# davidfang00/opticalflowdiffusion

Hardware: AMD Instinct MI355X
Metric: UNet denoise steps/sec @ 2x436x1024 flow, bs=16 (higher is better)
Workload: dtype bf16

## Files before the change

### opticalflowdiffusion_amd/build.py

```python
import concurrent.futures as cf
import os
import subprocess
import sys

HERE = os.path.dirname(os.path.abspath(__file__))
CSRC = os.path.join(HERE, "csrc")
OUT_DIR = os.path.join(HERE, "lib")
LIB = os.path.join(OUT_DIR, "libofd_hip.so")
ARCH = "gfx950"

COMMON = ["-O3", "-std=c++17", "-fPIC", f"--offload-arch={ARCH}", "-munsafe-fp-atomics",
          "-Wall", "-Wno-unused-function", "-Wno-unused-variable"]
EXTRA = {f: ["-ffp-contract=off"] for f in ("splat.hip", "grid_warp.hip", "splat_pyramid.hip", "diffusion.hip", "x0_quantile.hip",
                                                "loss_rows.hip")}


def sources():
    return sorted(f for f in os.listdir(CSRC) if f.endswith((".hip", ".cpp")))


def _deps_mtime():
    hdrs = [os.path.join(CSRC, f) for f in os.listdir(CSRC) if f.endswith((".h", ".hpp"))]
    hdrs.append(os.path.join(os.path.dirname(HERE), "include", "ofd.h"))
    return max(os.path.getmtime(h) for h in hdrs)


def _compile(src, force):
    obj = os.path.join(OUT_DIR, "obj", src + ".o")
    path = os.path.join(CSRC, src)
    if (not force and os.path.exists(obj) and os.path.getmtime(obj) > max(os.path.getmtime(path), _deps_mtime())):
        return obj, False
    cmd = ["hipcc", "-x", "hip", "-c", path, "-o", obj] + COMMON + EXTRA.get(src, [])
    r = subprocess.run(cmd, capture_output=True, text=True)
    if r.returncode != 0:
        raise RuntimeError(f"hipcc failed on {src}:\n{r.stdout}\n{r.stderr}")
    if r.stderr.strip():
        sys.stderr.write(r.stderr)
    return obj, True


def build(force=False, verbose=True):
    os.makedirs(os.path.join(OUT_DIR, "obj"), exist_ok=True)
    srcs = sources()
    with cf.ThreadPoolExecutor(max_workers=min(8, len(srcs))) as ex:
        results = list(ex.map(lambda s: _compile(s, force), srcs))
    objs = [o for o, _ in results]
    if any(c for _, c in results) or not os.path.exists(LIB):
        cmd = ["hipcc", "-shared", "-fPIC", f"--offload-arch={ARCH}", "-o", LIB] + objs
        r = subprocess.run(cmd, capture_output=True, text=True)
        if r.returncode != 0:
            raise RuntimeError(f"link failed:\n{r.stdout}\n{r.stderr}")
        if verbose:
            print(f"built {LIB} from {len(objs)} objects")
    return LIB


if __name__ == "__main__":
    build(force="--force" in sys.argv)
```

### opticalflowdiffusion_amd/csrc/blocks.hip

```cpp
#include <cstdlib>
#include "blocks.h"
#include "conv_common.h"

namespace ofd {

__device__ __forceinline__ uint32_t pack2(float a, float b) { return f2bf2(a, b); }
__device__ __forceinline__ void unpack8(const uint4& v, float (&f)[8]) {
    const uint32_t w[4] = {v.x, v.y, v.z, v.w};
#pragma unroll
    for (int j = 0; j < 4; ++j) {
        f[2 * j] = bf2f((bf16_t)(w[j] & 0xffffu));
        f[2 * j + 1] = bf2f((bf16_t)(w[j] >> 16));
    }
}
__device__ __forceinline__ uint4 pack8(const float (&f)[8]) {
    return make_uint4(pack2(f[0], f[1]), pack2(f[2], f[3]), pack2(f[4], f[5]), pack2(f[6], f[7]));
}

template <int CP>
__global__ void __launch_bounds__(256) pack_input_kernel(const float* __restrict__ x, int Cx, const float* __restrict__ cond, int Cc,
                                                         bf16_t* __restrict__ out, int B, size_t plane, int ax, int ac) {
    const size_t total = (size_t)B * plane;
    for (size_t i = (size_t)blockIdx.x * blockDim.x + threadIdx.x; i < total; i += (size_t)gridDim.x * blockDim.x) {
        const size_t n = i / plane, pix = i % plane;
        float v[CP];
#pragma unroll
        for (int c = 0; c < CP; ++c) {
            float t = 0.0f;
            if (c < Cx) { t = x[(n * Cx + c) * plane + pix]; if (ax) t = 2.0f * t - 1.0f; }
            else if (c < Cx + Cc) { t = cond[(n * Cc + (c - Cx)) * plane + pix]; if (ac) t = 2.0f * t - 1.0f; }
            v[c] = t;
        }
        uint4* o = (uint4*)(out + i * CP);
#pragma unroll
        for (int k = 0; k < CP / 8; ++k)
            o[k] = make_uint4(pack2(v[8 * k], v[8 * k + 1]), pack2(v[8 * k + 2], v[8 * k + 3]), pack2(v[8 * k + 4], v[8 * k + 5]), pack2(v[8 * k + 6], v[8 * k + 7]));
    }
}

__global__ void __launch_bounds__(256) time_mlp_kernel(const int64_t* __restrict__ t, const float* __restrict__ w1, const float* __restrict__ b1,
                                                       const float* __restrict__ w2, const float* __restrict__ b2, float* __restrict__ temb,
                                                       float* __restrict__ temb_silu, int dim) {
    __shared__ float emb[256], h1[1024];
    const int b = blockIdx.x, tid = threadIdx.x, tdim = dim * 4, half_dim = dim / 2;
    const float tv = (float)t[b];
    for (int i = tid; i < half_dim; i += 256) {
        const float k = (float)(9.210340371976184 / (double)(half_dim - 1));
        const float f = expf((float)i * -k);
        emb[i] = sinf(tv * f);
        emb[half_dim + i] = cosf(tv * f);
    }
    __syncthreads();
    for (int j = tid; j < tdim; j += 256) {
        float a = b1[j];
        for (int k = 0; k < dim; ++k) a += w1[(size_t)j * dim + k] * emb[k];
        h1[j] = 0.5f * a * (1.0f + erff(a * 0.70710678118654752f));
    }
    __syncthreads();
    for (int j = tid; j < tdim; j += 256) {
        float a = b2[j];
        for (int k = 0; k < tdim; ++k) a += w2[(size_t)j * tdim + k] * h1[k];
        temb[(size_t)b * tdim + j] = a;
        temb_silu[(size_t)b * tdim + j] = a / (1.0f + expf(-a));
    }
}

__global__ void __launch_bounds__(256) block_mlp_kernel(const float* __restrict__ temb_silu, const MlpDesc* __restrict__ descs,
                                                        float* __restrict__ ss, int tdim, int ss_stride) {
    __shared__ float e[1024];
    const int b = blockIdx.x, tid = threadIdx.x;
    const MlpDesc d = descs[blockIdx.y];
    for (int k = tid; k < tdim; k += 256) e[k] = temb_silu[(size_t)b * tdim + k];
    __syncthreads();
    for (int j = tid; j < d.n_out; j += 256) {
        float a = d.bias[j];
        const float* wr = d.weight + (size_t)j * tdim;
        if ((tdim & 3) == 0) {
#pragma unroll 8
            for (int k = 0; k < tdim; k += 4) {
                const float4 w4 = *(const float4*)(wr + k);
                a += w4.x * e[k];
                a += w4.y * e[k + 1];
                a += w4.z * e[k + 2];
                a += w4.w * e[k + 3];
            }
        } else {
            for (int k = 0; k < tdim; ++k) a += wr[k] * e[k];
        }
        ss[(size_t)b * ss_stride + d.offset + j] = a;
    }
}

constexpr int GNF_NT = 1024;
__global__ void __launch_bounds__(GNF_NT) gn_finalize_kernel(const float* __restrict__ partial, int tiles, int C, double count,
                                                          const float* __restrict__ gamma, const float* __restrict__ beta,
                                                          const float* __restrict__ ss, int ss_stride, int ss_offset,
                                                          float* __restrict__ a_out, float* __restrict__ s_out, float* __restrict__ stats_out) {
    const int b = blockIdx.x, g = blockIdx.y, tid = threadIdx.x;
    const int gs = C / 8, octs = gs / 8;
    constexpr int GU = 8;
    double s1 = 0.0, s2 = 0.0;
    const int total = tiles * octs;
    const float2* run = (const float2*)partial + ((size_t)b * 8 + g) * total;
    for (int i0 = tid; i0 < total; i0 += GNF_NT * GU) {
        float2 v[GU];
#pragma unroll
        for (int u = 0; u < GU; ++u) v[u] = run[min(i0 + u * GNF_NT, total - 1)];
#pragma unroll
        for (int u = 0; u < GU; ++u)
            if (i0 + u * GNF_NT < total) { s1 += (double)v[u].x; s2 += (double)v[u].y; }
    }
    for (int o = 32; o > 0; o >>= 1) { s1 += __shfl_xor(s1, o, 64); s2 += __shfl_xor(s2, o, 64); }
    __shared__ double r1[GNF_NT / 64], r2[GNF_NT / 64];
    if ((tid & 63) == 0) { r1[tid >> 6] = s1; r2[tid >> 6] = s2; }
    __syncthreads();
    for (int k = GNF_NT / 128; k > 0; k >>= 1) {
        if (tid < k) { r1[tid] += r1[tid + k]; r2[tid] += r2[tid + k]; }
        __syncthreads();
    }
    const double mean_d = r1[0] / count;
    double var_d = r2[0] / count - mean_d * mean_d;
    if (var_d < 0.0) var_d = 0.0;
    const float mean = (float)mean_d, rstd = rsqrtf((float)var_d + 1e-5f);
    if (stats_out && tid == 0) {
        stats_out[((size_t)b * 8 + g) * 2] = mean;
        stats_out[((size_t)b * 8 + g) * 2 + 1] = rstd;
    }
    for (int c = g * gs + tid; c < (g + 1) * gs; c += GNF_NT) {
        float sc = 0.0f, sh = 0.0f;
        if (ss) {
            sc = ss[(size_t)b * ss_stride + ss_offset + c];
            sh = ss[(size_t)b * ss_stride + ss_offset + C + c];
        }
        const float ga = gamma[c] * rstd;
        a_out[(size_t)b * C + c] = ga * (sc + 1.0f);
        s_out[(size_t)b * C + c] = (beta[c] - mean * ga) * (sc + 1.0f) + sh;
    }
}

__global__ void __launch_bounds__(256) resblock_out_kernel(const bf16_t* __restrict__ h, const float* __restrict__ a, const float* __restrict__ s,
                                                           const bf16_t* __restrict__ x, bf16_t* __restrict__ out, int C, size_t pix_per_sample, size_t total_units) {
    const int c8n = C / 8;
    for (size_t u = (size_t)blockIdx.x * blockDim.x + threadIdx.x; u < total_units; u += (size_t)gridDim.x * blockDim.x) {
        const size_t pix = u / c8n;
        const int c = (int)(u % c8n) * 8;
        const size_t b = pix / pix_per_sample;
        float hv[8], xv[8], av[8], sv[8];
        unpack8(*(const uint4*)(h + u * 8), hv);
        unpack8(*(const uint4*)(x + u * 8), xv);
        *(float4*)&av[0] = *(const float4*)(a + b * C + c);
        *(float4*)&av[4] = *(const float4*)(a + b * C + c + 4);
        *(float4*)&sv[0] = *(const float4*)(s + b * C + c);
        *(float4*)&sv[4] = *(const float4*)(s + b * C + c + 4);
#pragma unroll
        for (int j = 0; j < 8; ++j) hv[j] = silu_f(hv[j] * av[j] + sv[j]) + xv[j];
        *(uint4*)(out + u * 8) = pack8(hv);
    }
}

__global__ void __launch_bounds__(256) layernorm_c_kernel(const bf16_t* __restrict__ x, const float* __restrict__ g, const bf16_t* __restrict__ res,
                                                          bf16_t* __restrict__ out, int C, float eps, size_t npix) {
    const int lpp = C / 8;
    const int lane = threadIdx.x & 63;
    const int sub = lane % lpp, slot = lane / lpp, ppw = 64 / lpp;
    const size_t wave_global = ((size_t)blockIdx.x * blockDim.x + threadIdx.x) >> 6;
    const size_t nwaves = ((size_t)gridDim.x * blockDim.x) >> 6;
    float gv[8];
    *(float4*)&gv[0] = *(const float4*)(g + sub * 8);
    *(float4*)&gv[4] = *(const float4*)(g + sub * 8 + 4);
    const float inv_c = 1.0f / (float)C;
    for (size_t p0 = wave_global * ppw; p0 < npix; p0 += nwaves * ppw) {
        const size_t p = p0 + slot;
        const bool ok = p < npix;
        float v[8];
        if (ok) unpack8(*(const uint4*)(x + p * C + sub * 8), v);
        else {
#pragma unroll
            for (int j = 0; j < 8; ++j) v[j] = 0.0f;
        }
        float s = ((v[0] + v[1]) + (v[2] + v[3])) + ((v[4] + v[5]) + (v[6] + v[7]));
        for (int o = 1; o < lpp; o <<= 1) s += __shfl_xor(s, o, 64);
        const float mean = s * inv_c;
        float q = 0.0f;
#pragma unroll
        for (int j = 0; j < 8; ++j) { v[j] -= mean; q += v[j] * v[j]; }
        for (int o = 1; o < lpp; o <<= 1) q += __shfl_xor(q, o, 64);
        const float rstd = rsqrtf(q * inv_c + eps);
        if (ok) {
            float r[8];
            if (res) unpack8(*(const uint4*)(res + p * C + sub * 8), r);
#pragma unroll
            for (int j = 0; j < 8; ++j) v[j] = v[j] * rstd * gv[j] + (res ? r[j] : 0.0f);
            *(uint4*)(out + p * C + sub * 8) = pack8(v);
        }
    }
}

__global__ void __launch_bounds__(256) la_ctx_combine_kernel(const float* __restrict__ partial, float* __restrict__ ctx, int nparts, float inv_n, float* __restrict__ ml_out) {
    __shared__ float M[32], Linv[32], red[8][32];
    extern __shared__ float w_s[];
    const int tid = threadIdx.x, bh = blockIdx.x, dd = tid & 31, grp = tid >> 5;
    const float* base = partial + (size_t)bh * nparts * 1088;
    float mx = -3.0e38f;
    for (int c = grp; c < nparts; c += 8) mx = fmaxf(mx, base[(size_t)c * 1088 + dd]);
    red[grp][dd] = mx;
    __syncthreads();
    if (tid < 32) {
        float m = red[0][tid];
#pragma unroll
        for (int g = 1; g < 8; ++g) m = fmaxf(m, red[g][tid]);
        M[tid] = m;
    }
    __syncthreads();
    const bool use_ws = nparts <= 256;
    float l = 0.0f;
    for (int c = grp; c < nparts; c += 8) {
        const float w = __expf(base[(size_t)c * 1088 + dd] - M[dd]);
        if (use_ws) w_s[c * 32 + dd] = w;
        l += base[(size_t)c * 1088 + 32 + dd] * w;
    }
    __syncthreads();
    red[grp][dd] = l;
    __syncthreads();
    if (tid < 32) {
        float t = red[0][tid];
#pragma unroll
        for (int g = 1; g < 8; ++g) t += red[g][tid];
        Linv[tid] = 1.0f / t;
        if (ml_out && blockIdx.y == 0) {
            ml_out[(size_t)bh * 64 + tid] = M[tid];
            ml_out[(size_t)bh * 64 + 32 + tid] = 1.0f / t;
        }
    }
    __syncthreads();
    {
        const int i = blockIdx.y * 256 + tid, d = i >> 5;
        float a = 0.0f;
        for (int c0 = 0; c0 < nparts; c0 += 8) {
            float v[8];
#pragma unroll
            for (int k = 0; k < 8; ++k) v[k] = base[(size_t)min(c0 + k, nparts - 1) * 1088 + 64 + i];
            if (use_ws) {
#pragma unroll
                for (int k = 0; k < 8; ++k)
                    if (c0 + k < nparts) a += v[k] * w_s[(c0 + k) * 32 + d];
            } else {
#pragma unroll
                for (int k = 0; k < 8; ++k)
                    if (c0 + k < nparts) a += v[k] * __expf(base[(size_t)(c0 + k) * 1088 + d] - M[d]);
            }
        }
        ctx[(size_t)bh * 1024 + i] = a * Linv[d] * inv_n;
    }
}

constexpr int FA_KT = 64;
__global__ void __launch_bounds__(256) flash_attn_d32_kernel(const bf16_t* __restrict__ qkv, bf16_t* __restrict__ out, int n, float scale, float* __restrict__ lse) {
    __shared__ __attribute__((aligned(16))) unsigned char k_lds[FA_KT * 80];
    __shared__ __attribute__((aligned(16))) unsigned char vt_lds[32 * 144];
    const int tid = threadIdx.x, lane = tid & 63, wave = tid >> 6, l31 = lane & 31, half = lane >> 5;
    const int bh = blockIdx.y, b = bh / 4, h = bh % 4;
    const int q0 = blockIdx.x * 128 + wave * 32;
    const bf16_t* base = qkv + (size_t)b * n * 384;

    bf16x8 qf[2];
    {
        const int q = min(q0 + l31, n - 1);
#pragma unroll
        for (int s = 0; s < 2; ++s) qf[s] = *(const bf16x8*)(base + (size_t)q * 384 + h * 32 + s * 16 + half * 8);
    }
    f32x16 o_acc;
#pragma unroll
    for (int r = 0; r < 16; ++r) o_acc[r] = 0.0f;
    float m_run = -3.0e38f, l_run = 0.0f;

    for (int j0 = 0; j0 < n; j0 += FA_KT) {
        __syncthreads();
        {
            const int key = tid >> 2, u = tid & 3;
            const int kg = min(j0 + key, n - 1);
            const uint4 kv = *(const uint4*)(base + (size_t)kg * 384 + 128 + h * 32 + u * 8);
            *(uint4*)(k_lds + key * 80 + u * 16) = kv;
            const uint4 vv = *(const uint4*)(base + (size_t)kg * 384 + 256 + h * 32 + u * 8);
            const int kb = key >> 5, kk = key & 31, s = kk >> 4, a = (kk >> 3) & 1, hh = (kk >> 2) & 1, bb = kk & 3;
            const int slot = kb * 32 + s * 16 + hh * 8 + a * 4 + bb;
            const uint32_t w[4] = {vv.x, vv.y, vv.z, vv.w};
#pragma unroll
            for (int j = 0; j < 4; ++j) {
                *(bf16_t*)(vt_lds + (u * 8 + 2 * j) * 144 + slot * 2) = (bf16_t)(w[j] & 0xffffu);
                *(bf16_t*)(vt_lds + (u * 8 + 2 * j + 1) * 144 + slot * 2) = (bf16_t)(w[j] >> 16);
            }
        }
        __syncthreads();
        f32x16 s_acc[2];
#pragma unroll
        for (int kb = 0; kb < 2; ++kb) {
#pragma unroll
            for (int r = 0; r < 16; ++r) s_acc[kb][r] = 0.0f;
#pragma unroll
            for (int s = 0; s < 2; ++s) {
                const bf16x8 kf = *(const bf16x8*)(k_lds + (kb * 32 + l31) * 80 + (s * 16 + half * 8) * 2);
                s_acc[kb] = __builtin_amdgcn_mfma_f32_32x32x16_bf16(kf, qf[s], s_acc[kb], 0, 0, 0);
            }
        }
        if (j0 + FA_KT > n) {
#pragma unroll
            for (int kb = 0; kb < 2; ++kb)
#pragma unroll
                for (int r = 0; r < 16; ++r)
                    if (j0 + kb * 32 + (r & 3) + 8 * (r >> 2) + 4 * half >= n) s_acc[kb][r] = -3.0e38f;
        }
        float mx = -3.0e38f;
#pragma unroll
        for (int kb = 0; kb < 2; ++kb)
#pragma unroll
            for (int r = 0; r < 16; ++r) mx = fmaxf(mx, s_acc[kb][r]);
        mx = fmaxf(mx, __shfl_xor(mx, 32, 64));
        const float m_new = fmaxf(m_run, mx);
        const float c = scale * 1.4426950408889634f, m2 = m_new * c;
        const float alpha = __builtin_amdgcn_exp2f(__builtin_fmaf(m_run, c, -m2));
        m_run = m_new;
        float psum = 0.0f;
#pragma unroll
        for (int kb = 0; kb < 2; ++kb)
#pragma unroll
            for (int r = 0; r < 16; ++r) {
                const float p = __builtin_amdgcn_exp2f(__builtin_fmaf(s_acc[kb][r], c, -m2));
                s_acc[kb][r] = p;
                psum += p;
            }
        l_run = l_run * alpha + psum;
#pragma unroll
        for (int r = 0; r < 16; ++r) o_acc[r] *= alpha;
#pragma unroll
        for (int kb = 0; kb < 2; ++kb)
#pragma unroll
            for (int s = 0; s < 2; ++s) {
                bf16x8 pf;
#pragma unroll
                for (int j = 0; j < 8; ++j) pf[j] = (__bf16)s_acc[kb][8 * s + j];
                const bf16x8 vf = *(const bf16x8*)(vt_lds + l31 * 144 + (kb * 32 + s * 16 + half * 8) * 2);
                o_acc = __builtin_amdgcn_mfma_f32_32x32x16_bf16(vf, pf, o_acc, 0, 0, 0);
            }
    }
    const float l_tot = l_run + __shfl_xor(l_run, 32, 64);
    const float inv = 1.0f / l_tot;
    const int q = q0 + l31;
    if (lse && q < n && half == 0) lse[(size_t)bh * n + q] = m_run * scale + __logf(l_tot);
    if (q < n) {
        bf16_t* dst = out + ((size_t)b * n + q) * 128 + h * 32;
#pragma unroll
        for (int g = 0; g < 4; ++g) {
            const uint2 pk = make_uint2(pack2(o_acc[4 * g] * inv, o_acc[4 * g + 1] * inv), pack2(o_acc[4 * g + 2] * inv, o_acc[4 * g + 3] * inv));
            *(uint2*)(dst + 8 * g + 4 * half) = pk;
        }
    }
}

__device__ __forceinline__ float clamp1(float v) { return v < -1.0f ? -1.0f : (v > 1.0f ? 1.0f : v); }
__device__ __forceinline__ float out_glue(float v, int mode, float div) {
    if (mode == 1) return clamp1(clamp1(v) / div);
    if (mode == 2) return (clamp1(v) + 1.0f) / 2.0f;
    return v;
}

template <int OD>
__global__ void __launch_bounds__(256) final_conv_kernel(const bf16_t* __restrict__ x, const float* __restrict__ w, const float* __restrict__ bias,
                                                         float* __restrict__ out, int C, int out_dim, size_t plane, size_t total, int out_mode,
                                                         float out_div) {
    const int lpp = C / 8, lane = threadIdx.x & 63, sub = lane % lpp, slot = lane / lpp, ppw = 64 / lpp;
    float wv[OD][8];
#pragma unroll
    for (int o = 0; o < OD; ++o)
#pragma unroll
        for (int j = 0; j < 8; ++j) wv[o][j] = (o < out_dim) ? w[o * C + sub * 8 + j] : 0.0f;
    const size_t wave_global = ((size_t)blockIdx.x * blockDim.x + threadIdx.x) >> 6, nwaves = ((size_t)gridDim.x * blockDim.x) >> 6;
    for (size_t p0 = wave_global * ppw; p0 < total; p0 += nwaves * ppw) {
        const size_t i = min(p0 + slot, total - 1);
        float f[8];
        unpack8(*(const uint4*)(x + i * C + sub * 8), f);
        float acc[OD];
#pragma unroll
        for (int o = 0; o < OD; ++o) {
            acc[o] = 0.0f;
#pragma unroll
            for (int j = 0; j < 8; ++j) acc[o] += f[j] * wv[o][j];
            for (int k = 1; k < lpp; k <<= 1) acc[o] += __shfl_xor(acc[o], k, 64);
        }
        if (OD == 4) {
            if (sub < out_dim && p0 + slot < total) {
                const size_t n = i / plane, pix = i % plane;
                float r = acc[0];
                if (sub == 1) r = acc[1];
                if (sub == 2) r = acc[2];
                if (sub == 3) r = acc[3];
                out[(n * out_dim + sub) * plane + pix] = out_glue(r + bias[sub], out_mode, out_div);
            }
        } else if (p0 + slot < total) {
            const size_t n = i / plane, pix = i % plane;
#pragma unroll
            for (int o = 0; o < OD; ++o)
                if (o < out_dim && o % lpp == sub) out[(n * out_dim + o) * plane + pix] = out_glue(acc[o] + bias[o], out_mode, out_div);
        }
    }
}

__global__ void __launch_bounds__(256) nhwc_to_nchw_kernel(const bf16_t* __restrict__ x, float* __restrict__ out, int C, size_t plane, size_t total) {
    for (size_t i = (size_t)blockIdx.x * blockDim.x + threadIdx.x; i < total; i += (size_t)gridDim.x * blockDim.x) {
        const size_t pixc = i / C;
        const int c = (int)(i % C);
        const size_t n = pixc / plane, pix = pixc % plane;
        out[(n * C + c) * plane + pix] = bf2f(x[i]);
    }
}
__global__ void __launch_bounds__(256) nchw_to_nhwc_kernel(const float* __restrict__ x, bf16_t* __restrict__ out, int C, size_t plane, size_t total) {
    for (size_t i = (size_t)blockIdx.x * blockDim.x + threadIdx.x; i < total; i += (size_t)gridDim.x * blockDim.x) {
        const size_t pixc = i / C;
        const int c = (int)(i % C);
        const size_t n = pixc / plane, pix = pixc % plane;
        out[i] = f2bf(x[(n * C + c) * plane + pix]);
    }
}

static inline int sgrid(size_t total, int block = 256, int cap = 4096) {
    if (cap <= 0) cap = 1 << 22;
    size_t b = (total + block - 1) / block;
    return (int)(b < 1 ? 1 : (b > (size_t)cap ? cap : b));
}

int k_pack_input(const float* x, int Cx, const float* cond, int Cc, bf16_t* out, int B, int H, int W, hipStream_t s, int cpad, int ax, int ac) {
    OFD_CHECK_ARG((cpad == 8 || cpad == 16 || cpad == 32 || cpad == 48) && Cx + Cc <= cpad && Cx > 0, "pack_input: %d+%d channels into %d", Cx, Cc, cpad);
    const int g = sgrid((size_t)B * H * W);
    const size_t plane = (size_t)H * W;
    if (cpad == 8) pack_input_kernel<8><<<g, 256, 0, s>>>(x, Cx, cond, Cc, out, B, plane, ax, ac);
    else if (cpad == 16) pack_input_kernel<16><<<g, 256, 0, s>>>(x, Cx, cond, Cc, out, B, plane, ax, ac);
    else if (cpad == 32) pack_input_kernel<32><<<g, 256, 0, s>>>(x, Cx, cond, Cc, out, B, plane, ax, ac);
    else pack_input_kernel<48><<<g, 256, 0, s>>>(x, Cx, cond, Cc, out, B, plane, ax, ac);
    OFD_LAUNCH_CHECK();
    return OFD_OK;
}
int k_time_mlp(const int64_t* t, const float* w1, const float* b1, const float* w2, const float* b2, float* temb, float* temb_silu, int B, int dim, hipStream_t s) {
    OFD_CHECK_ARG(dim * 4 <= 1024 && dim <= 256, "time_mlp: dim %d too large", dim);
    time_mlp_kernel<<<B, 256, 0, s>>>(t, w1, b1, w2, b2, temb, temb_silu, dim);
    OFD_LAUNCH_CHECK();
    return OFD_OK;
}
int k_block_mlp(const float* temb_silu, const MlpDesc* descs, int n_desc, float* ss, int B, int tdim, int ss_stride, hipStream_t s) {
    block_mlp_kernel<<<dim3(B, n_desc), 256, 0, s>>>(temb_silu, descs, ss, tdim, ss_stride);
    OFD_LAUNCH_CHECK();
    return OFD_OK;
}
int k_gn_finalize(const float* partial, int B, int H, int W, int C, const float* gamma, const float* beta, const float* ss, int ss_stride,
                  int ss_offset, float* a_out, float* s_out, hipStream_t s, float* stats_out) {
    OFD_CHECK_ARG(C % 64 == 0, "gn_finalize: C=%d", C);
    const int tiles = cdiv(H, 8) * cdiv(W, 32) * 4;
    gn_finalize_kernel<<<dim3(B, 8), GNF_NT, 0, s>>>(partial, tiles, C, (double)H * W * (C / 8), gamma, beta, ss, ss_stride, ss_offset, a_out, s_out, stats_out);
    OFD_LAUNCH_CHECK();
    return OFD_OK;
}
int k_resblock_out(const bf16_t* h, const float* a, const float* sft, const bf16_t* x, bf16_t* out, int B, int H, int W, int C, hipStream_t s) {
    const size_t units = (size_t)B * H * W * (C / 8);
    resblock_out_kernel<<<sgrid(units, 256, 0), 256, 0, s>>>(h, a, sft, x, out, C, (size_t)H * W, units);
    OFD_LAUNCH_CHECK();
    return OFD_OK;
}
int k_layernorm_c(const bf16_t* x, const float* g, const bf16_t* res, bf16_t* out, size_t npix, int C, float eps, hipStream_t s) {
    OFD_CHECK_ARG(C == 64 || C == 128 || C == 256 || C == 512, "layernorm_c: C=%d unsupported", C);
    const size_t waves = (npix + (512 / C) - 1) / (512 / C);
    layernorm_c_kernel<<<sgrid(waves * 64, 256, 0), 256, 0, s>>>(x, g, res, out, C, eps, npix);
    OFD_LAUNCH_CHECK();
    return OFD_OK;
}
void launch_la_ctx_combine(const float* partial, float* ctx, int B, int nparts, float inv_n, float* ml_out, hipStream_t s) {
    const size_t lds = (size_t)(nparts <= 256 ? nparts : 1) * 32 * sizeof(float);
    la_ctx_combine_kernel<<<dim3(B * 4, 4), 256, lds, s>>>(partial, ctx, nparts, inv_n, ml_out);
}
int k_flash_attention(const bf16_t* qkv, bf16_t* out, int B, int n, hipStream_t s, float* lse) {
    flash_attn_d32_kernel<<<dim3(cdiv(n, 128), B * 4), 256, 0, s>>>(qkv, out, n, 0.17677669529663687f, lse);
    OFD_LAUNCH_CHECK();
    return OFD_OK;
}
int k_final_conv(const bf16_t* x, const float* w, const float* bias, float* out, int B, int H, int W, int C, int out_dim, hipStream_t s, int out_mode,
                 float out_div) {
    OFD_CHECK_ARG(out_dim >= 1 && out_dim <= 16 && C % 8 == 0, "final_conv: out_dim=%d C=%d", out_dim, C);
    OFD_CHECK_ARG(C == 64 || C == 128 || C == 256 || C == 512, "final_conv: C=%d unsupported", C);
    OFD_CHECK_ARG(out_mode >= 0 && out_mode <= 2 && out_div > 0.0f, "final_conv: out_mode=%d out_div=%g", out_mode, (double)out_div);
    const int g = sgrid(((size_t)B * H * W + (512 / C) - 1) / (512 / C) * 64);
    if (out_dim <= 4) final_conv_kernel<4><<<g, 256, 0, s>>>(x, w, bias, out, C, out_dim, (size_t)H * W, (size_t)B * H * W, out_mode, out_div);
    else final_conv_kernel<16><<<g, 256, 0, s>>>(x, w, bias, out, C, out_dim, (size_t)H * W, (size_t)B * H * W, out_mode, out_div);
    OFD_LAUNCH_CHECK();
    return OFD_OK;
}
int k_nhwc_to_nchw(const bf16_t* x, float* out, int B, int H, int W, int C, hipStream_t s) {
    const size_t total = (size_t)B * H * W * C;
    nhwc_to_nchw_kernel<<<sgrid(total), 256, 0, s>>>(x, out, C, (size_t)H * W, total);
    OFD_LAUNCH_CHECK();
    return OFD_OK;
}
int k_nchw_to_nhwc(const float* x, bf16_t* out, int B, int H, int W, int C, hipStream_t s) {
    const size_t total = (size_t)B * H * W * C;
    nchw_to_nhwc_kernel<<<sgrid(total), 256, 0, s>>>(x, out, C, (size_t)H * W, total);
    OFD_LAUNCH_CHECK();
    return OFD_OK;
}

}
```

Measured before the change: 34.31.

## Rewrite flash attention with double-buffered 128-key tiles and multi-query-block waves

Moves the d=32 flash attention kernel into its own file and restructures it. Key and value tiles are 128 keys wide and double-buffered in LDS, with global loads for the next tile issued before the current compute. That leaves one barrier per tile instead of two per 64 keys. V is stored in a permuted layout and read with a transpose-fragment helper instead of scalar transposing stores. Each wave can optionally process two 32-query blocks to reuse the K/V fragments, the rescale of the accumulator is skipped when the running max is unchanged, and P is packed to bf16 pairs directly. This adds LDS footprint and register pressure, and the grid-size heuristic picks NB=2 only in a narrow range.

```diff
diff --git a/opticalflowdiffusion_amd/build.py b/opticalflowdiffusion_amd/build.py
--- a/opticalflowdiffusion_amd/build.py
+++ b/opticalflowdiffusion_amd/build.py
@@ -13,6 +13,7 @@
           "-Wall", "-Wno-unused-function", "-Wno-unused-variable"]
 EXTRA = {f: ["-ffp-contract=off"] for f in ("splat.hip", "grid_warp.hip", "splat_pyramid.hip", "diffusion.hip", "x0_quantile.hip",
                                                 "loss_rows.hip")}
+EXTRA["flash_attn.hip"] = ["-fno-slp-vectorize"]
 
 
 def sources():
diff --git a/opticalflowdiffusion_amd/csrc/blocks.hip b/opticalflowdiffusion_amd/csrc/blocks.hip
--- a/opticalflowdiffusion_amd/csrc/blocks.hip
+++ b/opticalflowdiffusion_amd/csrc/blocks.hip
@@ -254,109 +254,6 @@
     }
 }
 
-constexpr int FA_KT = 64;
-__global__ void __launch_bounds__(256) flash_attn_d32_kernel(const bf16_t* __restrict__ qkv, bf16_t* __restrict__ out, int n, float scale, float* __restrict__ lse) {
-    __shared__ __attribute__((aligned(16))) unsigned char k_lds[FA_KT * 80];
-    __shared__ __attribute__((aligned(16))) unsigned char vt_lds[32 * 144];
-    const int tid = threadIdx.x, lane = tid & 63, wave = tid >> 6, l31 = lane & 31, half = lane >> 5;
-    const int bh = blockIdx.y, b = bh / 4, h = bh % 4;
-    const int q0 = blockIdx.x * 128 + wave * 32;
-    const bf16_t* base = qkv + (size_t)b * n * 384;
-
-    bf16x8 qf[2];
-    {
-        const int q = min(q0 + l31, n - 1);
-#pragma unroll
-        for (int s = 0; s < 2; ++s) qf[s] = *(const bf16x8*)(base + (size_t)q * 384 + h * 32 + s * 16 + half * 8);
-    }
-    f32x16 o_acc;
-#pragma unroll
-    for (int r = 0; r < 16; ++r) o_acc[r] = 0.0f;
-    float m_run = -3.0e38f, l_run = 0.0f;
-
-    for (int j0 = 0; j0 < n; j0 += FA_KT) {
-        __syncthreads();
-        {
-            const int key = tid >> 2, u = tid & 3;
-            const int kg = min(j0 + key, n - 1);
-            const uint4 kv = *(const uint4*)(base + (size_t)kg * 384 + 128 + h * 32 + u * 8);
-            *(uint4*)(k_lds + key * 80 + u * 16) = kv;
-            const uint4 vv = *(const uint4*)(base + (size_t)kg * 384 + 256 + h * 32 + u * 8);
-            const int kb = key >> 5, kk = key & 31, s = kk >> 4, a = (kk >> 3) & 1, hh = (kk >> 2) & 1, bb = kk & 3;
-            const int slot = kb * 32 + s * 16 + hh * 8 + a * 4 + bb;
-            const uint32_t w[4] = {vv.x, vv.y, vv.z, vv.w};
-#pragma unroll
-            for (int j = 0; j < 4; ++j) {
-                *(bf16_t*)(vt_lds + (u * 8 + 2 * j) * 144 + slot * 2) = (bf16_t)(w[j] & 0xffffu);
-                *(bf16_t*)(vt_lds + (u * 8 + 2 * j + 1) * 144 + slot * 2) = (bf16_t)(w[j] >> 16);
-            }
-        }
-        __syncthreads();
-        f32x16 s_acc[2];
-#pragma unroll
-        for (int kb = 0; kb < 2; ++kb) {
-#pragma unroll
-            for (int r = 0; r < 16; ++r) s_acc[kb][r] = 0.0f;
-#pragma unroll
-            for (int s = 0; s < 2; ++s) {
-                const bf16x8 kf = *(const bf16x8*)(k_lds + (kb * 32 + l31) * 80 + (s * 16 + half * 8) * 2);
-                s_acc[kb] = __builtin_amdgcn_mfma_f32_32x32x16_bf16(kf, qf[s], s_acc[kb], 0, 0, 0);
-            }
-        }
-        if (j0 + FA_KT > n) {
-#pragma unroll
-            for (int kb = 0; kb < 2; ++kb)
-#pragma unroll
-                for (int r = 0; r < 16; ++r)
-                    if (j0 + kb * 32 + (r & 3) + 8 * (r >> 2) + 4 * half >= n) s_acc[kb][r] = -3.0e38f;
-        }
-        float mx = -3.0e38f;
-#pragma unroll
-        for (int kb = 0; kb < 2; ++kb)
-#pragma unroll
-            for (int r = 0; r < 16; ++r) mx = fmaxf(mx, s_acc[kb][r]);
-        mx = fmaxf(mx, __shfl_xor(mx, 32, 64));
-        const float m_new = fmaxf(m_run, mx);
-        const float c = scale * 1.4426950408889634f, m2 = m_new * c;
-        const float alpha = __builtin_amdgcn_exp2f(__builtin_fmaf(m_run, c, -m2));
-        m_run = m_new;
-        float psum = 0.0f;
-#pragma unroll
-        for (int kb = 0; kb < 2; ++kb)
-#pragma unroll
-            for (int r = 0; r < 16; ++r) {
-                const float p = __builtin_amdgcn_exp2f(__builtin_fmaf(s_acc[kb][r], c, -m2));
-                s_acc[kb][r] = p;
-                psum += p;
-            }
-        l_run = l_run * alpha + psum;
-#pragma unroll
-        for (int r = 0; r < 16; ++r) o_acc[r] *= alpha;
-#pragma unroll
-        for (int kb = 0; kb < 2; ++kb)
-#pragma unroll
-            for (int s = 0; s < 2; ++s) {
-                bf16x8 pf;
-#pragma unroll
-                for (int j = 0; j < 8; ++j) pf[j] = (__bf16)s_acc[kb][8 * s + j];
-                const bf16x8 vf = *(const bf16x8*)(vt_lds + l31 * 144 + (kb * 32 + s * 16 + half * 8) * 2);
-                o_acc = __builtin_amdgcn_mfma_f32_32x32x16_bf16(vf, pf, o_acc, 0, 0, 0);
-            }
-    }
-    const float l_tot = l_run + __shfl_xor(l_run, 32, 64);
-    const float inv = 1.0f / l_tot;
-    const int q = q0 + l31;
-    if (lse && q < n && half == 0) lse[(size_t)bh * n + q] = m_run * scale + __logf(l_tot);
-    if (q < n) {
-        bf16_t* dst = out + ((size_t)b * n + q) * 128 + h * 32;
-#pragma unroll
-        for (int g = 0; g < 4; ++g) {
-            const uint2 pk = make_uint2(pack2(o_acc[4 * g] * inv, o_acc[4 * g + 1] * inv), pack2(o_acc[4 * g + 2] * inv, o_acc[4 * g + 3] * inv));
-            *(uint2*)(dst + 8 * g + 4 * half) = pk;
-        }
-    }
-}
-
 __device__ __forceinline__ float clamp1(float v) { return v < -1.0f ? -1.0f : (v > 1.0f ? 1.0f : v); }
 __device__ __forceinline__ float out_glue(float v, int mode, float div) {
     if (mode == 1) return clamp1(clamp1(v) / div);
@@ -475,11 +372,6 @@
     const size_t lds = (size_t)(nparts <= 256 ? nparts : 1) * 32 * sizeof(float);
     la_ctx_combine_kernel<<<dim3(B * 4, 4), 256, lds, s>>>(partial, ctx, nparts, inv_n, ml_out);
 }
-int k_flash_attention(const bf16_t* qkv, bf16_t* out, int B, int n, hipStream_t s, float* lse) {
-    flash_attn_d32_kernel<<<dim3(cdiv(n, 128), B * 4), 256, 0, s>>>(qkv, out, n, 0.17677669529663687f, lse);
-    OFD_LAUNCH_CHECK();
-    return OFD_OK;
-}
 int k_final_conv(const bf16_t* x, const float* w, const float* bias, float* out, int B, int H, int W, int C, int out_dim, hipStream_t s, int out_mode,
                  float out_div) {
     OFD_CHECK_ARG(out_dim >= 1 && out_dim <= 16 && C % 8 == 0, "final_conv: out_dim=%d C=%d", out_dim, C);
diff --git a/opticalflowdiffusion_amd/csrc/flash_attn.hip b/opticalflowdiffusion_amd/csrc/flash_attn.hip
--- /dev/null
+++ b/opticalflowdiffusion_amd/csrc/flash_attn.hip
@@ -0,0 +1,167 @@
+#include "blocks.h"
+#include "mfma_util.h"
+
+namespace ofd {
+
+constexpr int FA_KT = 128;
+constexpr int FA_KP = 80, FA_VP = 64;
+constexpr int FA_BUF = FA_KT * (FA_KP + FA_VP);
+
+__device__ __forceinline__ int fa_slot(int key) { return (key & ~12) | ((key & 4) << 1) | ((key & 8) >> 1); }
+
+template <int NB>
+__global__ void __launch_bounds__(256, 2) flash_attn_d32_kernel(const bf16_t* __restrict__ qkv, bf16_t* __restrict__ out, int n, float scale,
+                                                             float* __restrict__ lse) {
+    __shared__ __attribute__((aligned(16))) unsigned char smem[2 * FA_BUF];
+    const int tid = threadIdx.x, lane = tid & 63, wave = tid >> 6, l31 = lane & 31, half = lane >> 5;
+    const int bh = blockIdx.y, b = bh / 4, h = bh % 4;
+    const int q0 = blockIdx.x * (128 * NB) + wave * (32 * NB);
+    const bf16_t* base = qkv + (size_t)b * n * 384;
+
+    bf16x8 qf[NB][2];
+#pragma unroll
+    for (int blk = 0; blk < NB; ++blk) {
+        const int q = min(q0 + blk * 32 + l31, n - 1);
+#pragma unroll
+        for (int s = 0; s < 2; ++s) qf[blk][s] = *(const bf16x8*)(base + (size_t)q * 384 + h * 32 + s * 16 + half * 8);
+    }
+    f32x16 o_acc[NB];
+    float m_run[NB], l_run[NB];
+#pragma unroll
+    for (int blk = 0; blk < NB; ++blk) {
+#pragma unroll
+        for (int r = 0; r < 16; ++r) o_acc[blk][r] = 0.0f;
+        m_run[blk] = -3.0e38f;
+        l_run[blk] = 0.0f;
+    }
+
+    const int skey = tid >> 2, su = tid & 3;
+    const bf16_t* kv_src = base + 128 + h * 32 + su * 8;
+    const int k_off = skey * FA_KP + su * 16, v_off = FA_KT * FA_KP + fa_slot(skey) * FA_VP + su * 16;
+    uint4 kr0, kr1, vr0, vr1;
+#define FA_STAGE_LOAD(j0_)                                                                \
+    {                                                                                     \
+        const bf16_t* p0 = kv_src + (size_t)min((j0_) + skey, n - 1) * 384;               \
+        const bf16_t* p1 = kv_src + (size_t)min((j0_) + 64 + skey, n - 1) * 384;          \
+        kr0 = *(const uint4*)p0;                                                          \
+        vr0 = *(const uint4*)(p0 + 128);                                                  \
+        kr1 = *(const uint4*)p1;                                                          \
+        vr1 = *(const uint4*)(p1 + 128);                                                  \
+    }
+#define FA_STAGE_WRITE(buf_)                                                              \
+    {                                                                                     \
+        *(uint4*)((buf_) + k_off) = kr0;                                                  \
+        *(uint4*)((buf_) + v_off) = vr0;                                                  \
+        *(uint4*)((buf_) + 64 * FA_KP + k_off) = kr1;                                     \
+        *(uint4*)((buf_) + 64 * FA_VP + v_off) = vr1;                                     \
+    }
+    FA_STAGE_LOAD(0);
+    FA_STAGE_WRITE(smem);
+    __syncthreads();
+
+    const float c = scale * 1.4426950408889634f;
+    const int k_rd = l31 * FA_KP + half * 16;
+    for (int j0 = 0, cur = 0; j0 < n; j0 += FA_KT, cur ^= 1) {
+        const unsigned char* buf = smem + cur * FA_BUF;
+        const bool more = j0 + FA_KT < n;
+        if (more) FA_STAGE_LOAD(j0 + FA_KT);
+#pragma unroll
+        for (int hf = 0; hf < 2; ++hf) {
+            const int jh = j0 + hf * 64;
+            if (jh >= n) break;
+            bf16x8 kf[2][2], vf[2][2];
+#pragma unroll
+            for (int kb = 0; kb < 2; ++kb)
+#pragma unroll
+                for (int s = 0; s < 2; ++s) {
+                    kf[kb][s] = *(const bf16x8*)(buf + (hf * 64 + kb * 32) * FA_KP + k_rd + s * 32);
+                    vf[kb][s] = tr_frag(buf + FA_KT * FA_KP + (hf * 64 + kb * 32 + s * 16) * FA_VP, FA_VP, lane);
+                }
+#pragma unroll
+            for (int blk = 0; blk < NB; ++blk) {
+                if (blk > 0 && q0 + blk * 32 >= n) break;
+                f32x16 s_acc[2];
+#pragma unroll
+                for (int kb = 0; kb < 2; ++kb) {
+#pragma unroll
+                    for (int r = 0; r < 16; ++r) s_acc[kb][r] = 0.0f;
+#pragma unroll
+                    for (int s = 0; s < 2; ++s) s_acc[kb] = __builtin_amdgcn_mfma_f32_32x32x16_bf16(kf[kb][s], qf[blk][s], s_acc[kb], 0, 0, 0);
+                }
+                if (jh + 64 > n) {
+#pragma unroll
+                    for (int kb = 0; kb < 2; ++kb)
+#pragma unroll
+                        for (int r = 0; r < 16; ++r)
+                            if (jh + kb * 32 + (r & 3) + 8 * (r >> 2) + 4 * half >= n) s_acc[kb][r] = -3.0e38f;
+                }
+                float mx = fmaxf(s_acc[0][0], s_acc[1][0]);
+#pragma unroll
+                for (int r = 1; r < 16; ++r) mx = fmaxf(fmaxf(mx, s_acc[0][r]), s_acc[1][r]);
+                mx = fmaxf(mx, __shfl_xor(mx, 32, 64));
+                const float m_new = fmaxf(m_run[blk], mx);
+                const float m2 = m_new * c;
+                if (__ballot(m_new != m_run[blk]) != 0ull) {
+                    const float alpha = __builtin_amdgcn_exp2f(__builtin_fmaf(m_run[blk], c, -m2));
+                    m_run[blk] = m_new;
+                    l_run[blk] *= alpha;
+#pragma unroll
+                    for (int r = 0; r < 16; ++r) o_acc[blk][r] *= alpha;
+                }
+                float psum = 0.0f;
+                u32x4 pw[2][2];
+#pragma unroll
+                for (int kb = 0; kb < 2; ++kb)
+#pragma unroll
+                    for (int r = 0; r < 16; r += 2) {
+                        const float p0 = __builtin_amdgcn_exp2f(__builtin_fmaf(s_acc[kb][r], c, -m2));
+                        const float p1 = __builtin_amdgcn_exp2f(__builtin_fmaf(s_acc[kb][r + 1], c, -m2));
+                        psum += p0;
+                        psum += p1;
+                        pw[kb][r >> 3][(r & 7) >> 1] = f2bf2(p0, p1);
+                    }
+                l_run[blk] += psum;
+#pragma unroll
+                for (int kb = 0; kb < 2; ++kb)
+#pragma unroll
+                    for (int s = 0; s < 2; ++s)
+                        o_acc[blk] = __builtin_amdgcn_mfma_f32_32x32x16_bf16(vf[kb][s], __builtin_bit_cast(bf16x8, pw[kb][s]), o_acc[blk], 0, 0, 0);
+            }
+        }
+        if (more) FA_STAGE_WRITE(smem + (cur ^ 1) * FA_BUF);
+        __syncthreads();
+    }
+#undef FA_STAGE_LOAD
+#undef FA_STAGE_WRITE
+#pragma unroll
+    for (int blk = 0; blk < NB; ++blk) {
+        const float l_tot = l_run[blk] + __shfl_xor(l_run[blk], 32, 64);
+        const float inv = 1.0f / l_tot;
+        const int q = q0 + blk * 32 + l31;
+        if (lse && q < n && half == 0) lse[(size_t)bh * n + q] = m_run[blk] * scale + __logf(l_tot);
+        if (q < n) {
+            bf16_t* dst = out + ((size_t)b * n + q) * 128 + h * 32;
+#pragma unroll
+            for (int g = 0; g < 4; ++g) {
+                const uint2 pk = make_uint2(f2bf2(o_acc[blk][4 * g] * inv, o_acc[blk][4 * g + 1] * inv),
+                                            f2bf2(o_acc[blk][4 * g + 2] * inv, o_acc[blk][4 * g + 3] * inv));
+                *(uint2*)(dst + 8 * g + 4 * half) = pk;
+            }
+        }
+    }
+}
+
+static inline bool fa_two_blocks(int B, int n) {
+    const long wg2 = (long)cdiv(n, 256) * B * 4;
+    return wg2 >= 256 && wg2 <= 512;
+}
+
+int k_flash_attention(const bf16_t* qkv, bf16_t* out, int B, int n, hipStream_t s, float* lse) {
+    const float scale = 0.17677669529663687f;
+    if (fa_two_blocks(B, n)) flash_attn_d32_kernel<2><<<dim3(cdiv(n, 256), B * 4), 256, 0, s>>>(qkv, out, n, scale, lse);
+    else flash_attn_d32_kernel<1><<<dim3(cdiv(n, 128), B * 4), 256, 0, s>>>(qkv, out, n, scale, lse);
+    OFD_LAUNCH_CHECK();
+    return OFD_OK;
+}
+
+}
```

Measured after the change: 34.56 (median of 6 runs). About the same (+0.7%).
